# Veason-silverbullet/DIGAT

Hardware: AMD Instinct MI355X
Metric: MIND dev impressions scored/sec (AUC match not run) (higher is better)
Workload: dtype f32; 1 GPU; MIND-small default: --graph_encoder=DIGAT neighbors=3 hops=2 (N=10, U=67), d=400, graph_depth=3, fp32 dev inference; projection=auto -> fp16x3, N=10, U=67, d=400, graph_depth=3, news_num=65238, parallelism=dp1 (row shards, no data-path collective), ranks_in_process_group=1

## Files before the change

### digat_amd/csrc/digat_glue.inc

```

__global__ void __launch_bounds__(256) build_user_nodes_kernel(const float4* ue, const float4* topic, float4* Xu,
                                                               long B, int H, int C, int d4, const int* group, const uint8_t* rowmask = nullptr) {
    const long per_row = (long)(H + C) * d4;
    const long total = B * per_row;
    for (long i = (long)blockIdx.x * 256 + threadIdx.x; i < total; i += (long)gridDim.x * 256) {
        const long b = i / per_row;
        if (rowmask && rowmask[b] == 0) continue;
        const long rem = i - b * per_row;
        const long hist = (long)H * d4;
        const long src = group ? group[b] : b;
        Xu[i] = rem < hist ? ue[src * hist + rem] : topic[rem - hist];
    }
}

struct UserNodes3 { const float4* hist[3]; const float4* topic[3]; float4* dst[3]; };
__global__ void __launch_bounds__(256) build_user_nodes3_kernel(const UserNodes3 a, long B, int H, int C, int d4) {
    const int pl = blockIdx.y;
    const float4* ue = a.hist[pl];
    const float4* topic = a.topic[pl];
    float4* Xu = a.dst[pl];
    const long per_row = (long)(H + C) * d4;
    const long total = B * per_row;
    const long hist = (long)H * d4;
    for (long i = (long)blockIdx.x * 256 + threadIdx.x; i < total; i += (long)gridDim.x * 256) {
// ... 34 lines not shown
    unsigned long long col0 = 0ull, col1 = 0ull;
    unsigned long long own0[2] = {0ull, 0ull}, own1[2] = {0ull, 0ull};
    bool has0 = false, has1 = false;
    bool empty_row = false;
    int nz = 0;
    constexpr int RB = 8;
    for (int i0 = 0; i0 < U; i0 += RB) {
        uint8_t v0[RB], v1[RB];
#pragma unroll
        for (int r = 0; r < RB; ++r) {
            const uint8_t* row = A + (long)min(i0 + r, U - 1) * U;
            v0[r] = row[min(lane, U - 1)];
            v1[r] = row[min(lane + 64, U - 1)];
        }
#pragma unroll
        for (int r = 0; r < RB; ++r) {
            const int i = i0 + r;
            if (i >= U) break;
            unsigned long long m0 = __ballot(lane < U && v0[r] != 0), m1 = __ballot(lane + 64 < U && v1[r] != 0);
            nz += __popcll(m0) + __popcll(m1);
            empty_row |= (m0 | m1) == 0ull;
            if (twin && lane == (i & 63)) { own0[i >> 6] = m0; own1[i >> 6] = m1; }
            if (i < 64) m0 &= ~(1ull << i); else m1 &= ~(1ull << (i - 64));
            col0 |= m0; col1 |= m1;
            const bool has = (m0 | m1) != 0ull;
            if (lane == (i & 63)) { if (i < 64) has0 = has; else has1 = has; }
        }
    }
    const bool all_live = empty_row;
    int count = 0, last = 0;
    bool lv2[2] = {false, false};
#pragma unroll
    for (int h = 0; h < 2; ++h) {
        const int i = lane + 64 * h;
        bool live = false;
        if (i < U) {
            live = all_live || (h ? has1 : has0) || (((h ? col1 : col0) >> lane) & 1ull);
            if (i < H) {
                const long c = cat_idx[(long)b * H + i];
                live |= !any_cat || (c >= 0 && c < C1 && cat_mask[(long)b * C1 + c] != 0);
            }
            flags[(long)b * U + i] = live ? 1 : 0;
        }
        lv2[h] = live;
        count += __popcll(__ballot(live));
        const unsigned long long hm = __ballot(live && i < H);
        if (hm) last = 64 * h + 64 - __builtin_clzll(hm);
    }
    if (lane == 0) cnt[b] = count;
    if (lane == 0 && hlast) hlast[b] = last;
    if (twin) {
        int before[2] = {0, 0};
        unsigned word[2] = {0xFFFFFF00u | (unsigned)lane, 0xFFFFFF00u | (unsigned)(lane + 64)};
        unsigned long long rem0 = __ballot(lv2[0]), rem1 = __ballot(lv2[1]);
        while (rem0 | rem1) {
            const int hj = rem0 ? 0 : 1, lj = rem0 ? __builtin_ctzll(rem0) : __builtin_ctzll(rem1);
            const unsigned lo0 = (unsigned)__builtin_amdgcn_readlane((int)(unsigned)(hj ? own0[1] : own0[0]), lj);
            const unsigned hi0 = (unsigned)__builtin_amdgcn_readlane((int)(unsigned)((hj ? own0[1] : own0[0]) >> 32), lj);
            const unsigned lo1 = (unsigned)__builtin_amdgcn_readlane((int)(unsigned)(hj ? own1[1] : own1[0]), lj);
            const unsigned hi1 = (unsigned)__builtin_amdgcn_readlane((int)(unsigned)((hj ? own1[1] : own1[0]) >> 32), lj);
            const unsigned long long r0 = ((unsigned long long)hi0 << 32) | lo0, r1 = ((unsigned long long)hi1 << 32) | lo1;
            const bool e0 = lv2[0] && own0[0] == r0 && own1[0] == r1, e1 = lv2[1] && own0[1] == r0 && own1[1] == r1;
            const unsigned long long g0 = __ballot(e0), g1 = __ballot(e1);
            const unsigned long long below = (1ull << lane) - 1ull, above = lane == 63 ? 0ull : ~((2ull << lane) - 1ull);
            if (e0) {
                before[0] = __popcll(g0 & below);
                unsigned long long a0 = g0 & above, a1 = g1;
#pragma unroll
                for (int k = 1; k < TWIN_R; ++k) {
                    int j = -1;
                    if (a0) { j = __builtin_ctzll(a0); a0 &= a0 - 1ull; }
                    else if (a1) { j = 64 + __builtin_ctzll(a1); a1 &= a1 - 1ull; }
                    if (j >= 0) word[0] = (word[0] & ~(0xFFu << (8 * k))) | ((unsigned)j << (8 * k));
                }
            }
            if (e1) {
                before[1] = __popcll(g0) + __popcll(g1 & below);
                unsigned long long a1 = g1 & above;
#pragma unroll
                for (int k = 1; k < TWIN_R; ++k) {
                    if (a1) { const int j = 64 + __builtin_ctzll(a1); a1 &= a1 - 1ull; word[1] = (word[1] & ~(0xFFu << (8 * k))) | ((unsigned)j << (8 * k)); }
                }
            }
            rem0 &= ~g0; rem1 &= ~g1;
        }
        int leads = 0;
#pragma unroll
        for (int h = 0; h < 2; ++h) {
            const int i = lane + 64 * h;
            const bool lead = lv2[h] && (before[h] % TWIN_R) == 0;
            if (i < U) {
                twin[(long)b * U + i] = lead ? word[h] : 0xFFFFFFFFu;
                tflags[(long)b * U + i] = lead ? 1 : 0;
            }
            leads += __popcll(__ballot(lead));
        }
        if (lane == 0) tcnt[b] = leads;
    }
    if (entries && lane == 0) entries[b] = nz + (all_live ? U : 0);
    if (bflags) {
        int bc = 0;
        for (int c0 = 0; c0 < C1; c0 += 64) {
            const int c = c0 + lane;
            const bool bl = c < C1 && (!any_cat || cat_mask[(long)b * C1 + c] != 0);
            if (c < C1) bflags[(long)b * C1 + c] = bl ? 1 : 0;
            bc += __popcll(__ballot(bl));
        }
        if (lane == 0) bcnt[b] = bc;
    }
}

struct LiveExpand {
    const uint8_t* flags_g; const unsigned* twin_g; const uint8_t* tflags_g; const uint8_t* bflags_g;
    const int* cnt_g; const int* entries_g; const int* hlast_g; const int* bcnt_g; const int* tcnt_g;
    uint8_t* flags; unsigned* twin; uint8_t* tflags; uint8_t* bflags;
    int* cnt; int* entries; int* hlast; int* bcnt; int* tcnt;
};
__global__ void __launch_bounds__(256) live_expand_kernel(const LiveExpand a, const int* row_group, int B, int U, int C1) {
    const int lane = threadIdx.x & 63, wave = threadIdx.x >> 6;
    const int b = blockIdx.x * 4 + wave;
    if (b >= B) return;
    const long g = __builtin_amdgcn_readfirstlane(row_group[b]);
    if (a.flags_g == a.flags && g == b) return;
    for (int i = lane; i < U; i += 64) {
        a.flags[(long)b * U + i] = a.flags_g[g * U + i];
        if (a.twin) { a.twin[(long)b * U + i] = a.twin_g[g * U + i]; a.tflags[(long)b * U + i] = a.tflags_g[g * U + i]; }
    }
    if (a.bflags) for (int c = lane; c < C1; c += 64) a.bflags[(long)b * C1 + c] = a.bflags_g[g * C1 + c];
    if (lane == 0) {
        a.cnt[b] = a.cnt_g[g];
        if (a.hlast) a.hlast[b] = a.hlast_g[g];
        if (a.bcnt) a.bcnt[b] = a.bcnt_g[g];
        if (a.tcnt) a.tcnt[b] = a.tcnt_g[g];
        if (a.entries) a.entries[b] = a.entries_g[g];
    }
}

__global__ void __launch_bounds__(1024) sparse_decide_kernel(const int* entries, int B, int n, int per_node, int* flag) {
// ... 296 lines not shown
```

### digat_amd/csrc/digat_kernels.hip

```cpp
#include <hip/hip_runtime.h>
#include <stdint.h>
#include <string.h>
#include <stdlib.h>
#include <atomic>
#include <initializer_list>
#include <mutex>
#include <unordered_map>
#include <utility>

#include "../../include/digat_hip.h"
#include "digat_encoder_plan.h"

typedef float v4f __attribute__((ext_vector_type(4)));

#define DIGAT_CHECK_LAUNCH()                                   \
    do {                                                       \
        if (hipGetLastError() != hipSuccess) return DIGAT_ERR_LAUNCH; \
    } while (0)

static inline size_t align_up(size_t v, size_t a) { return (v + a - 1) / a * a; }
struct Arena {
    char* base; size_t cap, used; bool ok;
    Arena() : base(nullptr), cap(SIZE_MAX), used(0), ok(true) {}
    Arena(void* p, size_t n) : base((char*)p), cap(n), used(0), ok(p != nullptr) {}
// ... 65 lines not shown
    v += dpp_mov<0x141>(v);
    v += dpp_mov<0x140>(v);
#if DIGAT_WAVE_REDUCE_BCAST
    asm("s_nop 1\n\tv_add_f32_dpp %0, %0, %0 row_bcast:15 row_mask:0xa bank_mask:0xf\n\ts_nop 1\n\t"
        "v_add_f32_dpp %0, %0, %0 row_bcast:31 row_mask:0xc bank_mask:0xf\n\ts_nop 1" : "+v"(v));
    return lane_bcast(v, 63);
#else
    return (lane_bcast(v, 0) + lane_bcast(v, 16)) + (lane_bcast(v, 32) + lane_bcast(v, 48));
#endif
}
__device__ __forceinline__ float wave_max(float v) {
    v = fmaxf(v, dpp_mov<0xB1>(v));
    v = fmaxf(v, dpp_mov<0x4E>(v));
    v = fmaxf(v, dpp_mov<0x141>(v));
    v = fmaxf(v, dpp_mov<0x140>(v));
#if DIGAT_WAVE_REDUCE_BCAST
    asm("s_nop 1\n\tv_max_f32_dpp %0, %0, %0 row_bcast:15 row_mask:0xa bank_mask:0xf\n\ts_nop 1\n\t"
        "v_max_f32_dpp %0, %0, %0 row_bcast:31 row_mask:0xc bank_mask:0xf\n\ts_nop 1" : "+v"(v));
    return lane_bcast(v, 63);
#else
    return fmaxf(fmaxf(lane_bcast(v, 0), lane_bcast(v, 16)), fmaxf(lane_bcast(v, 32), lane_bcast(v, 48)));
#endif
}

__device__ __forceinline__ void lds_dma16(const float* gsrc, unsigned lds_byte_addr) {
    unsigned keep;
    asm volatile("s_mov_b32 %0, m0\n\ts_mov_b32 m0, %2\n\ts_nop 0\n\tglobal_load_lds_dwordx4 %1, off\n\ts_mov_b32 m0, %0"
                 : "=&s"(keep) : "v"(gsrc), "s"(lds_byte_addr) : "memory");
}
__device__ __forceinline__ void lds_dma16_s(const void* sbase_any, unsigned voff, unsigned lds_byte_addr) {
    const unsigned long long bits = (unsigned long long)(uintptr_t)sbase_any;
    const void* sbase = (const void*)(uintptr_t)(((unsigned long long)(unsigned)__builtin_amdgcn_readfirstlane((int)(bits >> 32)) << 32) |
                                                 (unsigned long long)(unsigned)__builtin_amdgcn_readfirstlane((int)bits));
    asm volatile("s_mov_b32 m0, %2\n\ts_nop 0\n\tglobal_load_lds_dwordx4 %0, %1" : : "v"(voff), "s"(sbase), "s"(lds_byte_addr) : "memory");
}
template <int N>
__device__ __forceinline__ void wait_vmcnt_imm() {
    __builtin_amdgcn_s_waitcnt((N & 15) | (7 << 4) | (15 << 8) | ((N >> 4) << 14));
}
__device__ __forceinline__ void wait_vmcnt(int n) {
    switch (n) {
        case 0: asm volatile("s_waitcnt vmcnt(0)" ::: "memory"); break;
        case 1: asm volatile("s_waitcnt vmcnt(1)" ::: "memory"); break;
        case 2: asm volatile("s_waitcnt vmcnt(2)" ::: "memory"); break;
        case 3: asm volatile("s_waitcnt vmcnt(3)" ::: "memory"); break;
        case 4: asm volatile("s_waitcnt vmcnt(4)" ::: "memory"); break;
        case 5: asm volatile("s_waitcnt vmcnt(5)" ::: "memory"); break;
        case 6: asm volatile("s_waitcnt vmcnt(6)" ::: "memory"); break;
        default: asm volatile("s_waitcnt vmcnt(4)" ::: "memory"); break;
    }
}

#ifndef DIGAT_TWIN_R
#define DIGAT_TWIN_R 2
#endif
__device__ __forceinline__ float leaky02_uniform(float e) {
    const float t = 0.2f * e;
    float r;
    asm("v_max_f32 %0, %1, %2" : "=v"(r) : "s"(e), "v"(t));
    return r;
}
__device__ __forceinline__ unsigned hash32(unsigned x) {
    x ^= x >> 16; x *= 0x7feb352dU; x ^= x >> 15; x *= 0x846ca68bU; x ^= x >> 16;
    return x;
}
__host__ __device__ __forceinline__ unsigned drop_threshold(float p) { return (unsigned)(p * 4294967296.0); }
__device__ __forceinline__ bool drop_keep(unsigned seed, long e, unsigned thr) {
    return hash32((unsigned)e * 0x9E3779B9U + hash32(seed + (unsigned)(e >> 32))) >= thr;
}
constexpr int TWIN_R = DIGAT_TWIN_R;
#include "digat_gemm.inc"
#include "digat_xattn.inc"
#include "digat_context.inc"
#include "digat_ctxfused.inc"
#include "digat_glue.inc"

extern "C" {

int digat_version(void) { return DIGAT_ABI_VERSION; }

const char* digat_error_string(int code) {
    switch (code) {
        case DIGAT_OK: return "ok";
        case DIGAT_ERR_ARG: return "bad argument (null pointer or negative size)";
        case DIGAT_ERR_SHAPE: return "unsupported shape (d % 4 != 0, graph larger than DIGAT_MAX_NODES, depth too large)";
        case DIGAT_ERR_WORKSPACE: return "workspace too small";
        case DIGAT_ERR_LAUNCH: return "HIP kernel launch failed";
        default: return "unknown error";
    }
}

int digat_linear_f32(const float* x, int64_t ldx, const float* w, const float* b, float* y, int64_t ldy,
                     int M, int N, int K, void* stream) {
    if (!x || !w || !y || M < 0 || N <= 0 || K <= 0) return DIGAT_ERR_ARG;
    if (K % 4 || ldx % 4) return DIGAT_ERR_SHAPE;
    return launch_gemm(gemm_plain(x, ldx, w, b, y, ldy, M, N, K, 0), (hipStream_t)stream);
}

struct XattnWs { float *h, *P, *Q, *r, *alpha; };
static XattnWs xattn_carve(Arena& a, int B, int n, int d) {
    const size_t nd = (size_t)B * n * d;
    XattnWs w{};
    w.h = a.take<float>(3 * nd);
    if (w.h) { w.P = w.h + nd; w.Q = w.P + nd; }
    w.r = a.take<float>((size_t)B * d);
    w.alpha = a.take<float>((size_t)B * n * n);
    return w;
}
size_t digat_xattn_workspace_bytes(int B, int n, int d) { Arena a; xattn_carve(a, B, n, d); return a.used; }

int digat_xattn_pairwise_fwd(const float* Pr, const float* Q, const float* h, const float* X,
                             const float* a, const uint8_t* A, float* out, float* alpha,
                             int B, int n, int d, void* stream) {
    if (!Pr || !Q || !h || !X || !a || !A || !out || !alpha) return DIGAT_ERR_ARG;
    return launch_xattn_pairwise(Pr, Q, h, X, a, A, out, alpha, B, n, d, (hipStream_t)stream);
}

struct TwinLists { const unsigned* word; const int* list; const int* count; };

struct XattnOpts {
    const void* wsplit = nullptr;
    const int* rowidx = nullptr; const int* nrows_dev = nullptr; const uint8_t* live = nullptr;
    int sparse_mode = DIGAT_XATTN_DENSE; const int* sparse_flag = nullptr;
// ... 512 lines not shown
```

### digat_amd/csrc/digat_xattn.inc

```

struct ScoreArgs {
    const float* P;
    const float* Q; const float* a; const uint8_t* A; float* alpha;
    float* s_out;
    const uint8_t* live;
    const int* qgroup;
    const float* radd;
    const int64_t* bindex;
    const float* agg_h; const float* agg_x; float* agg_out;
    int B, n, d, d4;
    int NT, SN, CC4, nchunks, RB;
    int img_slots;
    int ring_slots;
    int ninstr;
    int am_off;
    int a_off;
    int tl_off;
    int ld_off;
    int pm_off;
    const int* skip_if;
    uint8_t* amask; float* adrop; float drop_p; unsigned drop_seed;
};
constexpr int XA_RING = 3;
constexpr int XA_KMAX = 4;
// ... 966 lines not shown
#pragma unroll
        for (int u = 0; u < U; ++u) acc[r][u] = f4_zero();
    {
        unsigned long long m0 = m[0], m1 = m[1];
        while (m0 | m1) {
            int j[NBR], cnt = 0;
#pragma unroll
            for (int t = 0; t < NBR; ++t) {
                if (m0) { j[t] = __builtin_ctzll(m0); m0 &= m0 - 1ull; ++cnt; }
                else if (m1) { j[t] = 64 + __builtin_ctzll(m1); m1 &= m1 - 1ull; ++cnt; }
                else j[t] = j[0];
            }
            float4 hv[NBR][U];
#pragma unroll
            for (int t = 0; t < NBR; ++t)
#pragma unroll
                for (int u = 0; u < U; ++u) hv[t][u] = (Hb + (long)j[t] * d4)[c4l[u]];
#pragma unroll
            for (int t = 0; t < NBR; ++t) {
                if (t < cnt) {
#pragma unroll
                    for (int r = 0; r < R; ++r) {
                        if (r < nr) {
                            const float w = j[t] < 64 ? lane_bcast(al[r][0], j[t]) : lane_bcast(al[r][1], j[t] - 64);
#pragma unroll
                            for (int u = 0; u < U; ++u) {
                                acc[r][u].x = fmaf(w, hv[t][u].x, acc[r][u].x); acc[r][u].y = fmaf(w, hv[t][u].y, acc[r][u].y);
                                acc[r][u].z = fmaf(w, hv[t][u].z, acc[r][u].z); acc[r][u].w = fmaf(w, hv[t][u].w, acc[r][u].w);
                            }
                        }
                    }
                }
            }
        }
    }
#pragma unroll
    for (int r = 0; r < R; ++r) {
        if (r < nr) {
            float4* Oi = reinterpret_cast<float4*>(g.out) + (rho + (long)r * n) * d4;
#pragma unroll
            for (int u = 0; u < U; ++u) {
                const int c4 = lane + 64 * u;
                if (c4 < d4) {
                    const float4 x = xin[u];
                    const float4 o = make_float4(fmaxf(acc[r][u].x, 0.f) + x.x, fmaxf(acc[r][u].y, 0.f) + x.y,
                                                 fmaxf(acc[r][u].z, 0.f) + x.z, fmaxf(acc[r][u].w, 0.f) + x.w);
                    Oi[c4] = o;
                }
            }
        }
    }
}

template <int U, int R>
__device__ __forceinline__ void xattn_sparse_twin_chunk(const SparseArgs& g, const long rho, const unsigned word, const uint8_t ab0, const uint8_t ab1,
                                                        const int lane) {
    constexpr int NBR = DIGAT_SPARSE_NBR;
    const int n = g.n, d4 = g.d4;
    const long b = rho / n;
    int mem[R], nr = 0;
#pragma unroll
    for (int r = 0; r < R; ++r) {
        const int mi = (int)((word >> (8 * r)) & 0xFFu);
        const bool ok = mi != 0xFF && (g.centre_limit <= 0 || mi < g.centre_limit);
        mem[r] = ok ? mi : mem[0];
        nr += ok ? 1 : 0;
        if (r == 0 && !ok) return;
    }
    const float4* a4 = reinterpret_cast<const float4*>(g.a);
    float4 av[U], q[R][U];
    unsigned c4l[U];
#pragma unroll
    for (int u = 0; u < U; ++u) {
        const int c4 = min(lane + 64 * u, d4 - 1);
        c4l[u] = (unsigned)c4;
        const float4 aa = a4[c4];
        av[u] = lane + 64 * u < d4 ? aa : f4_zero();
#pragma unroll
        for (int r = 0; r < R; ++r) q[r][u] = reinterpret_cast<const float4*>(g.Q)[(b * n + mem[r]) * d4 + c4];
    }
    const float4* Pb = reinterpret_cast<const float4*>(g.P) + b * n * d4;
    const float4* Hb = reinterpret_cast<const float4*>(g.h) + b * n * d4;
    unsigned long long m[2];
    m[0] = __ballot(lane < n && ab0 != 0);
    m[1] = __ballot(lane + 64 < n && ab1 != 0);
    const int deg = __popcll(m[0]) + __popcll(m[1]);
    float al[R][2];
    if (deg == 0) {
        m[0] = n >= 64 ? ~0ull : ((1ull << n) - 1ull);
        m[1] = n > 64 ? (n >= 128 ? ~0ull : ((1ull << (n - 64)) - 1ull)) : 0ull;
        const float w = 1.f / (float)n;
#pragma unroll
        for (int r = 0; r < R; ++r) { al[r][0] = lane < n ? w : 0.f; al[r][1] = lane + 64 < n ? w : 0.f; }
    } else if (deg == 1) {
#pragma unroll
        for (int r = 0; r < R; ++r) { al[r][0] = ((m[0] >> lane) & 1ull) ? 1.f : 0.f; al[r][1] = ((m[1] >> lane) & 1ull) ? 1.f : 0.f; }
    } else {
        float sc[R][2];
#pragma unroll
        for (int r = 0; r < R; ++r) { sc[r][0] = -INFINITY; sc[r][1] = -INFINITY; }
        unsigned long long m0 = m[0], m1 = m[1];
        while (m0 | m1) {
            int j[NBR], cnt = 0;
#pragma unroll
            for (int t = 0; t < NBR; ++t) {
                if (m0) { j[t] = __builtin_ctzll(m0); m0 &= m0 - 1ull; ++cnt; }
                else if (m1) { j[t] = 64 + __builtin_ctzll(m1); m1 &= m1 - 1ull; ++cnt; }
                else j[t] = j[0];
            }
            float4 p[NBR][U];
#pragma unroll
            for (int t = 0; t < NBR; ++t)
#pragma unroll
                for (int u = 0; u < U; ++u) p[t][u] = (Pb + (long)j[t] * d4)[c4l[u]];
#pragma unroll
            for (int t = 0; t < NBR; ++t) {
                if (t < cnt) {
#pragma unroll
                    for (int r = 0; r < R; ++r) {
                        if (r < nr) {
                            float part = 0.f;
#pragma unroll
                            for (int u = 0; u < U; ++u) {
                                const float4 pk = p[t][u];
                                part = fmaf(av[u].x, fmaxf(pk.x + q[r][u].x, 0.f), part);
                                part = fmaf(av[u].y, fmaxf(pk.y + q[r][u].y, 0.f), part);
                                part = fmaf(av[u].z, fmaxf(pk.z + q[r][u].z, 0.f), part);
                                part = fmaf(av[u].w, fmaxf(pk.w + q[r][u].w, 0.f), part);
                            }
                            const float e = wave_sum(part);
                            const float lk = leaky02_uniform(e);
                            if (lane == (j[t] & 63)) { if (j[t] < 64) sc[r][0] = lk; else sc[r][1] = lk; }
                        }
                    }
                }
            }
        }
#pragma unroll
        for (int r = 0; r < R; ++r) {
            const float mx = wave_max(fmaxf(sc[r][0], sc[r][1]));
            const float e0 = sc[r][0] > -INFINITY ? expf(sc[r][0] - mx) : 0.f;
            const float e1 = sc[r][1] > -INFINITY ? expf(sc[r][1] - mx) : 0.f;
            const float inv = wave_sum(e0 + e1);
            al[r][0] = e0 / inv;
            al[r][1] = e1 / inv;
        }
    }
    float4 xin[R][U];
    {
        unsigned xo[U];
#pragma unroll
        for (int u = 0; u < U; ++u) { xo[u] = c4l[u]; asm volatile("" : "+v"(xo[u]) : "v"(al[0][0])); }
#pragma unroll
        for (int u = 0; u < U; ++u) xin[0][u] = reinterpret_cast<const float4*>(g.X)[(b * n + mem[0]) * d4 + xo[u]];
    }
    float4 acc[R][U];
#pragma unroll
    for (int r = 0; r < R; ++r)
#pragma unroll
        for (int u = 0; u < U; ++u) acc[r][u] = f4_zero();
    {
        unsigned long long m0 = m[0], m1 = m[1];
        while (m0 | m1) {
            int j[NBR], cnt = 0;
#pragma unroll
            for (int t = 0; t < NBR; ++t) {
                if (m0) { j[t] = __builtin_ctzll(m0); m0 &= m0 - 1ull; ++cnt; }
                else if (m1) { j[t] = 64 + __builtin_ctzll(m1); m1 &= m1 - 1ull; ++cnt; }
                else j[t] = j[0];
            }
            float4 hv[NBR][U];
#pragma unroll
            for (int t = 0; t < NBR; ++t)
#pragma unroll
                for (int u = 0; u < U; ++u) hv[t][u] = (Hb + (long)j[t] * d4)[c4l[u]];
#pragma unroll
            for (int t = 0; t < NBR; ++t) {
                if (t < cnt) {
#pragma unroll
                    for (int r = 0; r < R; ++r) {
                        if (r < nr) {
                            const float w = j[t] < 64 ? lane_bcast(al[r][0], j[t]) : lane_bcast(al[r][1], j[t] - 64);
#pragma unroll
                            for (int u = 0; u < U; ++u) {
                                acc[r][u].x = fmaf(w, hv[t][u].x, acc[r][u].x); acc[r][u].y = fmaf(w, hv[t][u].y, acc[r][u].y);
                                acc[r][u].z = fmaf(w, hv[t][u].z, acc[r][u].z); acc[r][u].w = fmaf(w, hv[t][u].w, acc[r][u].w);
                            }
                        }
                    }
                }
            }
        }
    }
    if (nr > 1) {
#pragma unroll
        for (int r = 1; r < R; ++r)
#pragma unroll
            for (int u = 0; u < U; ++u) xin[r][u] = reinterpret_cast<const float4*>(g.X)[(b * n + mem[r]) * d4 + c4l[u]];
    }
#pragma unroll
    for (int r = 0; r < R; ++r) {
        if (r < nr) {
            float4* Oi = reinterpret_cast<float4*>(g.out) + (b * n + mem[r]) * d4;
#pragma unroll
            for (int u = 0; u < U; ++u) {
                const int c4 = lane + 64 * u;
                if (c4 < d4) {
                    const float4 x = xin[r][u];
                    const float4 o = make_float4(fmaxf(acc[r][u].x, 0.f) + x.x, fmaxf(acc[r][u].y, 0.f) + x.y,
                                                 fmaxf(acc[r][u].z, 0.f) + x.z, fmaxf(acc[r][u].w, 0.f) + x.w);
                    Oi[c4] = o;
                }
            }
        }
    }
}

#ifndef DIGAT_TWIN_WAVES
#define DIGAT_TWIN_WAVES (DIGAT_TWIN_R <= 2 ? 5 : 4)
#endif
#ifndef DIGAT_TWIN_WPG
#define DIGAT_TWIN_WPG 4
#endif
template <int U, int R>
__global__ void __launch_bounds__(64 * DIGAT_TWIN_WPG, U <= 2 ? DIGAT_TWIN_WAVES : 1) xattn_sparse_twin_kernel(const SparseArgs g) {
    const int lane = threadIdx.x & 63, wave = __builtin_amdgcn_readfirstlane(threadIdx.x >> 6);
    if (g.exec_rows && g.exec_unit && blockIdx.x == 0 && threadIdx.x == 0) atomicAdd(g.exec_rows, (unsigned long long)*g.nrows_dev * g.exec_unit);
    unsigned blk = blockIdx.x;
    if (g.xcd_group > 0) {
        const unsigned Gx = (unsigned)g.xcd_group, w = blk / (8 * Gx), r = blk - w * 8 * Gx;
        blk = w * 8 * Gx + (r & 7) * Gx + (r >> 3);
    }
    const long count = *g.twcount;
    const long stride = (long)gridDim.x * DIGAT_TWIN_WPG;
    long k = (long)blk * DIGAT_TWIN_WPG + wave;
    if (k >= count) return;
    const int n = g.n;
    long rho = __builtin_amdgcn_readfirstlane(g.twlist[k]);
    unsigned word_v = g.twin[rho];
    uint8_t ab0 = g.A[rho * n + min(lane, n - 1)], ab1 = g.A[rho * n + min(lane + 64, n - 1)];
    int rho_next_v = g.twlist[min(k + stride, count - 1)];
    for (;;) {
        const long kn = k + stride;
        const bool more = kn < count;
        const long rho_n = more ? (long)__builtin_amdgcn_readfirstlane(rho_next_v) : rho;
        const unsigned word_n = g.twin[rho_n];
        const uint8_t ab0_n = g.A[rho_n * n + min(lane, n - 1)], ab1_n = g.A[rho_n * n + min(lane + 64, n - 1)];
        rho_next_v = g.twlist[min(kn + stride, count - 1)];
        xattn_sparse_twin_chunk<U, R>(g, rho, (unsigned)__builtin_amdgcn_readfirstlane((int)word_v), ab0, ab1, lane);
        if (!more) break;
        k = kn; rho = rho_n; word_v = word_n; ab0 = ab0_n; ab1 = ab1_n;
    }
}

__global__ void __launch_bounds__(1024) sparse_count_kernel(const int* rowidx, const int* nrows_dev, int n, int limit, unsigned unit, unsigned unit_nbr,
                                                            unsigned long long* out) {
    __shared__ int part[16], part2[16];
    const int total = *nrows_dev;
    int lo = 0, hi = 0;
    for (int k = blockIdx.x * 1024 + threadIdx.x; k < total; k += gridDim.x * 1024) { lo += (rowidx[k] % n) < limit; ++hi; }
    for (int o = 32; o > 0; o >>= 1) { lo += __shfl_xor(lo, o, 64); hi += __shfl_xor(hi, o, 64); }
    if ((threadIdx.x & 63) == 0) { part[threadIdx.x >> 6] = lo; part2[threadIdx.x >> 6] = hi; }
    __syncthreads();
    if (threadIdx.x == 0) {
        long t = 0, m = 0;
        for (int w = 0; w < 16; ++w) { t += part[w]; m += part2[w]; }
        if (m) atomicAdd(out, (unsigned long long)t * unit + (unsigned long long)(m - t) * unit_nbr);
    }
}

__global__ void __launch_bounds__(1024) sparse_l0_bytes_kernel(const uint8_t* live, const int* row_group, int B, int n, unsigned row_bytes,
                                                               unsigned long long* out) {
    __shared__ unsigned long long part[16];
    unsigned long long c = 0;
    for (int b = blockIdx.x * 1024 + threadIdx.x; b < B; b += gridDim.x * 1024) {
        int lv = 0;
        for (int i = 0; i < n; ++i) lv += live[(long)b * n + i] != 0;
        const bool first = b == 0 || row_group[b] != row_group[b - 1];
        c += (unsigned long long)lv * row_bytes + (first ? (unsigned long long)lv * (4ull * row_bytes + n) : 0ull);
    }
    for (int o = 32; o > 0; o >>= 1) c += __shfl_xor(c, o, 64);
    if ((threadIdx.x & 63) == 0) part[threadIdx.x >> 6] = c;
    __syncthreads();
    if (threadIdx.x == 0) {
        unsigned long long t = 0;
        for (int w = 0; w < 16; ++w) t += part[w];
        atomicAdd(out, t);
    }
}

static double sparse_bytes(const SparseArgs& g) {
    const double row = (double)g.d4 * 16;
    if (g.rowidx) return row + (g.radd ? (double)g.B * row : 0.0);
    double bytes = (double)g.B * g.n * g.n + row + (g.radd ? (double)g.B * row : 0.0);
    const double rows_b = (double)g.B * g.n, rows_g = (double)(g.group && g.G > 0 ? g.G : g.B) * g.n;
    bytes += 3.0 * rows_g * row;
    bytes += (g.group && g.xgroup ? rows_g : rows_b) * row;
    bytes += rows_b * row;
    return bytes;
}
static int sparse_part(const SparseArgs& g) { return g.prof_part ? g.prof_part - 1 : (g.rowidx ? (g.group ? XPART_L0 : XPART_TWIN) : XPART_OTHER); }
static int sparse_prof_bytes(SparseArgs& g, hipStream_t st) {
    g.exec_rows = nullptr; g.exec_unit = 0;
    if (!g.rowidx || !g_prof.enabled || !((g_prof.kind_mask >> DIGAT_KERNEL_XATTN) & 1u)) return DIGAT_OK;
    const unsigned row = (unsigned)g.d4 * 16;
    g.exec_rows = g_prof.rows_dev + 8 + sparse_part(g);
    const unsigned unit = g.pq16 == 2 ? (unsigned)(3.5 * row + 2.0 * 4 * (g.d4 / 20) + g.n) : (g.pq16 ? 4u : 5u) * row + (unsigned)g.n;
    if (g.group && g.live && !g.prof_part) {
        hipLaunchKernelGGL(sparse_l0_bytes_kernel, dim3((g.B + 1023) / 1024), dim3(1024), 0, st, g.live, g.group, g.B, g.n, row, g.exec_rows);
        DIGAT_CHECK_LAUNCH();
    } else if (g.centre_limit > 0) {
        hipLaunchKernelGGL(sparse_count_kernel, dim3(64), dim3(1024), 0, st, g.rowidx, g.nrows_dev, g.n, g.centre_limit, unit,
                           g.pq16 ? row + row / (g.pq16 == 2 ? 4 : 2) : 2 * row, g.exec_rows);
        DIGAT_CHECK_LAUNCH();
    } else {
        g.exec_unit = unit;
    }
    return DIGAT_OK;
}

#ifdef DIGAT_SPARSE_TIMERS
static unsigned long long* g_sparse_timers = nullptr;
extern "C" int digat_debug_sparse_timers(double* out9) {
    if (!g_sparse_timers || !out9) return DIGAT_ERR_ARG;
    unsigned long long h[9];
    if (hipDeviceSynchronize() != hipSuccess || hipMemcpy(h, g_sparse_timers, sizeof(h), hipMemcpyDeviceToHost) != hipSuccess) return DIGAT_ERR_LAUNCH;
    for (int k = 0; k < 9; ++k) out9[k] = (double)h[k];
    (void)hipMemset(g_sparse_timers, 0, 16 * 8);
    return DIGAT_OK;
}
#endif
static int launch_sparse(const SparseArgs& g_in, hipStream_t st) {
    SparseArgs g = g_in;
    if (g.n > 128 || g.d4 > 256) return DIGAT_ERR_SHAPE;
    { const int rcp = sparse_prof_bytes(g, st); if (rcp) return rcp; }
    ProfScope prof(DIGAT_KERNEL_XATTN, sparse_bytes(g), st, 0.0, sparse_part(g));
    unsigned blocks = (unsigned)(((long)g.B * g.n + 3) / 4);
    if (g.run_if && blocks > 2048u) blocks = 2048u;
    constexpr int SPARSE_XCD_GROUP = 16;
    g.xcd_group = SPARSE_XCD_GROUP;
#ifdef DIGAT_SPARSE_TIMERS
    if (!g_sparse_timers && hipMalloc((void**)&g_sparse_timers, 16 * 8) == hipSuccess) (void)hipMemset(g_sparse_timers, 0, 16 * 8);
    g.timers = g.rowidx ? g_sparse_timers : nullptr;
#endif
    blocks = (blocks + 8u * g.xcd_group - 1) / (8u * g.xcd_group) * (8u * g.xcd_group);
    if (g.twin && g.twlist && g.twcount && g.rowidx && !g.pq16 && !g.radd && !g.group && !g.run_if && !g.fill_flags && g.d4 <= 128) {
        constexpr unsigned TWIN_GRID_CAP = 8192;
        if (blocks > TWIN_GRID_CAP) blocks = TWIN_GRID_CAP;
        blocks = (blocks * 4 + DIGAT_TWIN_WPG - 1) / DIGAT_TWIN_WPG;
        if (g.d4 <= 64) hipLaunchKernelGGL((xattn_sparse_twin_kernel<1, TWIN_R>), dim3(blocks), dim3(64 * DIGAT_TWIN_WPG), 0, st, g);
        else hipLaunchKernelGGL((xattn_sparse_twin_kernel<2, TWIN_R>), dim3(blocks), dim3(64 * DIGAT_TWIN_WPG), 0, st, g);
        DIGAT_CHECK_LAUNCH();
        return DIGAT_OK;
    }
    if (g.pq16 == 2) {
        if (g.radd || g.d4 % 20 || g.ld8 < 4 * g.d4 + 4 * (g.d4 / 20) || (g.ld8 & 7)) return DIGAT_ERR_SHAPE;
        if (g.d4 <= 64) hipLaunchKernelGGL((xattn_sparse_kernel<1, 2, false>), dim3(blocks), dim3(256), 0, st, g);
        else if (g.d4 <= 128) hipLaunchKernelGGL((xattn_sparse_kernel<2, 2, false>), dim3(blocks), dim3(256), 0, st, g);
        else hipLaunchKernelGGL((xattn_sparse_kernel<4, 2, false>), dim3(blocks), dim3(256), 0, st, g);
    } else if (g.pq16) {
        if (g.radd || (g.d4 & 1)) return DIGAT_ERR_SHAPE;
        if (g.d4 <= 64) hipLaunchKernelGGL((xattn_sparse_kernel<1, 1, false>), dim3(blocks), dim3(256), 0, st, g);
        else if (g.d4 <= 128) hipLaunchKernelGGL((xattn_sparse_kernel<2, 1, false>), dim3(blocks), dim3(256), 0, st, g);
        else hipLaunchKernelGGL((xattn_sparse_kernel<4, 1, false>), dim3(blocks), dim3(256), 0, st, g);
    } else if (g.radd) {
        if (g.d4 <= 64) hipLaunchKernelGGL((xattn_sparse_kernel<1, 0, true>), dim3(blocks), dim3(256), 0, st, g);
        else if (g.d4 <= 128) hipLaunchKernelGGL((xattn_sparse_kernel<2, 0, true>), dim3(blocks), dim3(256), 0, st, g);
        else hipLaunchKernelGGL((xattn_sparse_kernel<4, 0, true>), dim3(blocks), dim3(256), 0, st, g);
    } else {
        if (g.d4 <= 64) hipLaunchKernelGGL((xattn_sparse_kernel<1, 0, false>), dim3(blocks), dim3(256), 0, st, g);
        else if (g.d4 <= 128) hipLaunchKernelGGL((xattn_sparse_kernel<2, 0, false>), dim3(blocks), dim3(256), 0, st, g);
        else hipLaunchKernelGGL((xattn_sparse_kernel<4, 0, false>), dim3(blocks), dim3(256), 0, st, g);
    }
    DIGAT_CHECK_LAUNCH();
    return DIGAT_OK;
}

#ifndef DIGAT_L0_ROWS
#define DIGAT_L0_ROWS 4
#endif
constexpr int SPARSE_L0_ROWS = DIGAT_L0_ROWS;
static bool sparse_l0_ok(const SparseArgs& g) {
    return g.group && g.xgroup && g.radd && g.rowidx && g.nrows_dev && g.live && !g.run_if && !g.pq16 && !g.fill_flags && !g.centre_limit &&
           g.n <= 128 && g.d4 <= 128;
}
static int launch_sparse_l0(const SparseArgs& g_in, const uint8_t* lead, const int* list, const int* count, int G, hipStream_t st) {
    SparseL0Args a{g_in, lead, list, count};
    SparseArgs& g = a.g;
    { const int rcp = sparse_prof_bytes(g, st); if (rcp) return rcp; }
    ProfScope prof(DIGAT_KERNEL_XATTN, sparse_bytes(g), st, 0.0, XPART_L0);
    constexpr int L0_XCD_GROUP = 16;
    g.xcd_group = L0_XCD_GROUP;
    unsigned blocks = (unsigned)((((long)g.B / SPARSE_L0_ROWS + G) * g.n + 3) / 4);
    blocks = (blocks + 8u * g.xcd_group - 1) / (8u * g.xcd_group) * (8u * g.xcd_group);
    if (g.d4 <= 64) hipLaunchKernelGGL((xattn_sparse_l0_kernel<1, SPARSE_L0_ROWS>), dim3(blocks), dim3(256), 0, st, a);
    else hipLaunchKernelGGL((xattn_sparse_l0_kernel<2, SPARSE_L0_ROWS>), dim3(blocks), dim3(256), 0, st, a);
    DIGAT_CHECK_LAUNCH();
    return DIGAT_OK;
}

struct AggArgs {
    const float* alpha; const float* Hh; const float* X; float* out; int B, n, d, groups, sa;
    const uint8_t* live;
    const int* hgroup;
// ... 219 lines not shown
```

Measured before the change: 39100 impressions/s.

## Group non-history twin rows with differing adjacency and raise twin group size

Rows at index H and above (topic/candidate nodes) are now grouped into twin chunks regardless of adjacency equality and flagged with a high bit. A uniform-adjacency-free variant of the sparse twin chunk then computes per-row masks and degrees and scores the union of neighbours. TWIN_R goes from 2 to 4 so more rows share the loaded P/H neighbour rows. Loads switch to scalar-base plus vector-offset addressing, and the neighbour batch sizes become template parameters. The aim is more reuse of each neighbour fetch per wave, at the cost of extra register pressure and wasted work on neighbours that only some rows in the group use.

```diff
diff --git a/digat_amd/csrc/digat_glue.inc b/digat_amd/csrc/digat_glue.inc
--- a/digat_amd/csrc/digat_glue.inc
+++ b/digat_amd/csrc/digat_glue.inc
@@ -110,7 +110,32 @@
     if (twin) {
         int before[2] = {0, 0};
         unsigned word[2] = {0xFFFFFF00u | (unsigned)lane, 0xFFFFFF00u | (unsigned)(lane + 64)};
-        unsigned long long rem0 = __ballot(lv2[0]), rem1 = __ballot(lv2[1]);
+        const unsigned long long below = (1ull << lane) - 1ull, above = lane == 63 ? 0ull : ~((2ull << lane) - 1ull);
+        auto place = [&](const bool e0, const bool e1, const unsigned long long g0, const unsigned long long g1) {
+            if (e0) {
+                before[0] = __popcll(g0 & below);
+                unsigned long long a0 = g0 & above, a1 = g1;
+#pragma unroll
+                for (int k = 1; k < TWIN_R; ++k) {
+                    int j = -1;
+                    if (a0) { j = __builtin_ctzll(a0); a0 &= a0 - 1ull; }
+                    else if (a1) { j = 64 + __builtin_ctzll(a1); a1 &= a1 - 1ull; }
+                    if (j >= 0) word[0] = (word[0] & ~(0xFFu << (8 * k))) | ((unsigned)j << (8 * k));
+                }
+            }
+            if (e1) {
+                before[1] = __popcll(g0) + __popcll(g1 & below);
+                unsigned long long a1 = g1 & above;
+#pragma unroll
+                for (int k = 1; k < TWIN_R; ++k) {
+                    if (a1) { const int j = 64 + __builtin_ctzll(a1); a1 &= a1 - 1ull; word[1] = (word[1] & ~(0xFFu << (8 * k))) | ((unsigned)j << (8 * k)); }
+                }
+            }
+        };
+        const bool top0 = lv2[0] && lane >= H, top1 = lv2[1] && lane + 64 >= H;
+        const unsigned long long t0 = __ballot(top0), t1 = __ballot(top1);
+        place(top0, top1, t0, t1);
+        unsigned long long rem0 = __ballot(lv2[0]) & ~t0, rem1 = __ballot(lv2[1]) & ~t1;
         while (rem0 | rem1) {
             const int hj = rem0 ? 0 : 1, lj = rem0 ? __builtin_ctzll(rem0) : __builtin_ctzll(rem1);
             const unsigned lo0 = (unsigned)__builtin_amdgcn_readlane((int)(unsigned)(hj ? own0[1] : own0[0]), lj);
@@ -118,30 +143,13 @@
             const unsigned lo1 = (unsigned)__builtin_amdgcn_readlane((int)(unsigned)(hj ? own1[1] : own1[0]), lj);
             const unsigned hi1 = (unsigned)__builtin_amdgcn_readlane((int)(unsigned)((hj ? own1[1] : own1[0]) >> 32), lj);
             const unsigned long long r0 = ((unsigned long long)hi0 << 32) | lo0, r1 = ((unsigned long long)hi1 << 32) | lo1;
-            const bool e0 = lv2[0] && own0[0] == r0 && own1[0] == r1, e1 = lv2[1] && own0[1] == r0 && own1[1] == r1;
+            const bool e0 = lv2[0] && !top0 && own0[0] == r0 && own1[0] == r1, e1 = lv2[1] && !top1 && own0[1] == r0 && own1[1] == r1;
             const unsigned long long g0 = __ballot(e0), g1 = __ballot(e1);
-            const unsigned long long below = (1ull << lane) - 1ull, above = lane == 63 ? 0ull : ~((2ull << lane) - 1ull);
-            if (e0) {
-                before[0] = __popcll(g0 & below);
-                unsigned long long a0 = g0 & above, a1 = g1;
-#pragma unroll
-                for (int k = 1; k < TWIN_R; ++k) {
-                    int j = -1;
-                    if (a0) { j = __builtin_ctzll(a0); a0 &= a0 - 1ull; }
-                    else if (a1) { j = 64 + __builtin_ctzll(a1); a1 &= a1 - 1ull; }
-                    if (j >= 0) word[0] = (word[0] & ~(0xFFu << (8 * k))) | ((unsigned)j << (8 * k));
-                }
-            }
-            if (e1) {
-                before[1] = __popcll(g0) + __popcll(g1 & below);
-                unsigned long long a1 = g1 & above;
-#pragma unroll
-                for (int k = 1; k < TWIN_R; ++k) {
-                    if (a1) { const int j = 64 + __builtin_ctzll(a1); a1 &= a1 - 1ull; word[1] = (word[1] & ~(0xFFu << (8 * k))) | ((unsigned)j << (8 * k)); }
-                }
-            }
+            place(e0, e1, g0, g1);
             rem0 &= ~g0; rem1 &= ~g1;
         }
+        if (top0 && (word[0] >> 8) != 0xFFFFFFu) word[0] |= 0x80u;
+        if (top1 && (word[1] >> 8) != 0xFFFFFFu) word[1] |= 0x80u;
         int leads = 0;
 #pragma unroll
         for (int h = 0; h < 2; ++h) {
diff --git a/digat_amd/csrc/digat_kernels.hip b/digat_amd/csrc/digat_kernels.hip
--- a/digat_amd/csrc/digat_kernels.hip
+++ b/digat_amd/csrc/digat_kernels.hip
@@ -141,7 +141,13 @@
 }
 
 #ifndef DIGAT_TWIN_R
-#define DIGAT_TWIN_R 2
+#define DIGAT_TWIN_R 4
+#endif
+#ifndef DIGAT_TWIN_NBR
+#define DIGAT_TWIN_NBR 2
+#endif
+#ifndef DIGAT_TWIN_NBR_AGG
+#define DIGAT_TWIN_NBR_AGG DIGAT_TWIN_NBR
 #endif
 __device__ __forceinline__ float leaky02_uniform(float e) {
     const float t = 0.2f * e;
@@ -158,6 +164,7 @@
     return hash32((unsigned)e * 0x9E3779B9U + hash32(seed + (unsigned)(e >> 32))) >= thr;
 }
 constexpr int TWIN_R = DIGAT_TWIN_R;
+constexpr int TWIN_NBR = DIGAT_TWIN_NBR, TWIN_NBR_AGG = DIGAT_TWIN_NBR_AGG;
 #include "digat_gemm.inc"
 #include "digat_xattn.inc"
 #include "digat_context.inc"
diff --git a/digat_amd/csrc/digat_xattn.inc b/digat_amd/csrc/digat_xattn.inc
--- a/digat_amd/csrc/digat_xattn.inc
+++ b/digat_amd/csrc/digat_xattn.inc
@@ -1042,17 +1042,35 @@
     }
 }
 
-template <int U, int R>
+typedef float f4raw __attribute__((ext_vector_type(4)));
+__device__ __forceinline__ float4 row_piece(const float4* row, const unsigned byte_off) {
+    unsigned long long base = reinterpret_cast<unsigned long long>(row);
+    asm("" : "+s"(base));
+    unsigned off = byte_off;
+    asm volatile("" : "+v"(off));
+    const auto* gb = reinterpret_cast<const __attribute__((address_space(1))) char*>(base);
+    const f4raw v = *reinterpret_cast<const __attribute__((address_space(1))) f4raw*>(gb + off);
+    return make_float4(v[0], v[1], v[2], v[3]);
+}
+__device__ __forceinline__ void row_piece_store(float4* row, const unsigned byte_off, const float4 v) {
+    unsigned long long base = reinterpret_cast<unsigned long long>(row);
+    asm("" : "+s"(base));
+    unsigned off = byte_off;
+    asm volatile("" : "+v"(off));
+    auto* gb = reinterpret_cast<__attribute__((address_space(1))) char*>(base);
+    const f4raw w = {v.x, v.y, v.z, v.w};
+    *reinterpret_cast<__attribute__((address_space(1))) f4raw*>(gb + off) = w;
+}
+template <int U, int R, int NBR, int NBRA, bool UNI>
 __device__ __forceinline__ void xattn_sparse_twin_chunk(const SparseArgs& g, const long rho, const unsigned word, const uint8_t ab0, const uint8_t ab1,
                                                         const int lane) {
-    constexpr int NBR = DIGAT_SPARSE_NBR;
     const int n = g.n, d4 = g.d4;
     const long b = rho / n;
     int mem[R], nr = 0;
 #pragma unroll
     for (int r = 0; r < R; ++r) {
-        const int mi = (int)((word >> (8 * r)) & 0xFFu);
-        const bool ok = mi != 0xFF && (g.centre_limit <= 0 || mi < g.centre_limit);
+        const int mi = (int)((word >> (8 * r)) & (r == 0 ? 0x7Fu : 0xFFu));
+        const bool ok = (r == 0 || mi != 0xFF) && (g.centre_limit <= 0 || mi < g.centre_limit);
         mem[r] = ok ? mi : mem[0];
         nr += ok ? 1 : 0;
         if (r == 0 && !ok) return;
@@ -1060,36 +1078,46 @@
     const float4* a4 = reinterpret_cast<const float4*>(g.a);
     float4 av[U], q[R][U];
     unsigned c4l[U];
+    uint8_t mb[UNI ? R : 1][2];
+    if constexpr (UNI) {
+#pragma unroll
+        for (int r = 1; r < R; ++r) {
+            const uint8_t* Ar = g.A + (b * n + mem[r]) * n;
+            mb[r][0] = Ar[min(lane, n - 1)]; mb[r][1] = Ar[min(lane + 64, n - 1)];
+        }
+    }
 #pragma unroll
     for (int u = 0; u < U; ++u) {
-        const int c4 = min(lane + 64 * u, d4 - 1);
-        c4l[u] = (unsigned)c4;
-        const float4 aa = a4[c4];
+        c4l[u] = 16u * (unsigned)min(lane + 64 * u, d4 - 1);
+        const float4 aa = row_piece(a4, c4l[u]);
         av[u] = lane + 64 * u < d4 ? aa : f4_zero();
 #pragma unroll
-        for (int r = 0; r < R; ++r) q[r][u] = reinterpret_cast<const float4*>(g.Q)[(b * n + mem[r]) * d4 + c4];
+        for (int r = 0; r < R; ++r) q[r][u] = row_piece(reinterpret_cast<const float4*>(g.Q) + (b * n + mem[r]) * d4, c4l[u]);
     }
     const float4* Pb = reinterpret_cast<const float4*>(g.P) + b * n * d4;
     const float4* Hb = reinterpret_cast<const float4*>(g.h) + b * n * d4;
-    unsigned long long m[2];
-    m[0] = __ballot(lane < n && ab0 != 0);
-    m[1] = __ballot(lane + 64 < n && ab1 != 0);
-    const int deg = __popcll(m[0]) + __popcll(m[1]);
+    constexpr int RM = UNI ? R : 1;
+    unsigned long long mk[RM][2];
+    int deg[RM];
+    unsigned long long su[2] = {0ull, 0ull};
+#pragma unroll
+    for (int r = 0; r < RM; ++r) {
+        const uint8_t b0 = r == 0 ? ab0 : mb[r][0], b1 = r == 0 ? ab1 : mb[r][1];
+        const bool in = r < nr;
+        mk[r][0] = in ? __ballot(lane < n && b0 != 0) : 0ull;
+        mk[r][1] = in ? __ballot(lane + 64 < n && b1 != 0) : 0ull;
+        deg[r] = in ? __popcll(mk[r][0]) + __popcll(mk[r][1]) : 2;
+        if (deg[r] >= 2) { su[0] |= mk[r][0]; su[1] |= mk[r][1]; }
+    }
+    auto takes = [&](const int r, const int j, const bool scoring) -> bool {
+        if constexpr (UNI) return (!scoring || deg[r] >= 2) && ((j < 64 ? mk[r][0] >> j : mk[r][1] >> (j - 64)) & 1ull) != 0ull;
+        else return r < nr;
+    };
     float al[R][2];
-    if (deg == 0) {
-        m[0] = n >= 64 ? ~0ull : ((1ull << n) - 1ull);
-        m[1] = n > 64 ? (n >= 128 ? ~0ull : ((1ull << (n - 64)) - 1ull)) : 0ull;
-        const float w = 1.f / (float)n;
-#pragma unroll
-        for (int r = 0; r < R; ++r) { al[r][0] = lane < n ? w : 0.f; al[r][1] = lane + 64 < n ? w : 0.f; }
-    } else if (deg == 1) {
-#pragma unroll
-        for (int r = 0; r < R; ++r) { al[r][0] = ((m[0] >> lane) & 1ull) ? 1.f : 0.f; al[r][1] = ((m[1] >> lane) & 1ull) ? 1.f : 0.f; }
-    } else {
-        float sc[R][2];
-#pragma unroll
-        for (int r = 0; r < R; ++r) { sc[r][0] = -INFINITY; sc[r][1] = -INFINITY; }
-        unsigned long long m0 = m[0], m1 = m[1];
+#pragma unroll
+    for (int r = 0; r < R; ++r) { al[r][0] = -INFINITY; al[r][1] = -INFINITY; }
+    {
+        unsigned long long m0 = su[0], m1 = su[1];
         while (m0 | m1) {
             int j[NBR], cnt = 0;
 #pragma unroll
@@ -1102,13 +1130,13 @@
 #pragma unroll
             for (int t = 0; t < NBR; ++t)
 #pragma unroll
-                for (int u = 0; u < U; ++u) p[t][u] = (Pb + (long)j[t] * d4)[c4l[u]];
+                for (int u = 0; u < U; ++u) p[t][u] = row_piece(Pb + (long)j[t] * d4, c4l[u]);
 #pragma unroll
             for (int t = 0; t < NBR; ++t) {
                 if (t < cnt) {
 #pragma unroll
                     for (int r = 0; r < R; ++r) {
-                        if (r < nr) {
+                        if (takes(r, j[t], true)) {
                             float part = 0.f;
 #pragma unroll
                             for (int u = 0; u < U; ++u) {
@@ -1120,20 +1148,30 @@
                             }
                             const float e = wave_sum(part);
                             const float lk = leaky02_uniform(e);
-                            if (lane == (j[t] & 63)) { if (j[t] < 64) sc[r][0] = lk; else sc[r][1] = lk; }
+                            if (lane == (j[t] & 63)) { if (j[t] < 64) al[r][0] = lk; else al[r][1] = lk; }
                         }
                     }
                 }
             }
         }
-#pragma unroll
-        for (int r = 0; r < R; ++r) {
-            const float mx = wave_max(fmaxf(sc[r][0], sc[r][1]));
-            const float e0 = sc[r][0] > -INFINITY ? expf(sc[r][0] - mx) : 0.f;
-            const float e1 = sc[r][1] > -INFINITY ? expf(sc[r][1] - mx) : 0.f;
-            const float inv = wave_sum(e0 + e1);
-            al[r][0] = e0 / inv;
-            al[r][1] = e1 / inv;
+    }
+#pragma unroll
+    for (int r = 0; r < R; ++r) {
+        if (r < nr) {
+            const int rm = UNI ? r : 0;
+            if (deg[rm] == 0) {
+                const float w = 1.f / (float)n;
+                al[r][0] = lane < n ? w : 0.f; al[r][1] = lane + 64 < n ? w : 0.f;
+            } else if (deg[rm] == 1) {
+                al[r][0] = ((mk[rm][0] >> lane) & 1ull) ? 1.f : 0.f; al[r][1] = ((mk[rm][1] >> lane) & 1ull) ? 1.f : 0.f;
+            } else {
+                const float mx = wave_max(fmaxf(al[r][0], al[r][1]));
+                const float e0 = al[r][0] > -INFINITY ? expf(al[r][0] - mx) : 0.f;
+                const float e1 = al[r][1] > -INFINITY ? expf(al[r][1] - mx) : 0.f;
+                const float inv = wave_sum(e0 + e1);
+                al[r][0] = e0 / inv;
+                al[r][1] = e1 / inv;
+            }
         }
     }
     float4 xin[R][U];
@@ -1142,34 +1180,43 @@
 #pragma unroll
         for (int u = 0; u < U; ++u) { xo[u] = c4l[u]; asm volatile("" : "+v"(xo[u]) : "v"(al[0][0])); }
 #pragma unroll
-        for (int u = 0; u < U; ++u) xin[0][u] = reinterpret_cast<const float4*>(g.X)[(b * n + mem[0]) * d4 + xo[u]];
+        for (int u = 0; u < U; ++u) xin[0][u] = row_piece(reinterpret_cast<const float4*>(g.X) + (b * n + mem[0]) * d4, xo[u]);
     }
     float4 acc[R][U];
 #pragma unroll
     for (int r = 0; r < R; ++r)
 #pragma unroll
         for (int u = 0; u < U; ++u) acc[r][u] = f4_zero();
+    unsigned long long au[2] = {0ull, 0ull};
+#pragma unroll
+    for (int r = 0; r < RM; ++r) {
+        if (deg[r] == 0) {
+            mk[r][0] = n >= 64 ? ~0ull : ((1ull << n) - 1ull);
+            mk[r][1] = n > 64 ? (n >= 128 ? ~0ull : ((1ull << (n - 64)) - 1ull)) : 0ull;
+        }
+        au[0] |= mk[r][0]; au[1] |= mk[r][1];
+    }
     {
-        unsigned long long m0 = m[0], m1 = m[1];
+        unsigned long long m0 = au[0], m1 = au[1];
         while (m0 | m1) {
-            int j[NBR], cnt = 0;
-#pragma unroll
-            for (int t = 0; t < NBR; ++t) {
+            int j[NBRA], cnt = 0;
+#pragma unroll
+            for (int t = 0; t < NBRA; ++t) {
                 if (m0) { j[t] = __builtin_ctzll(m0); m0 &= m0 - 1ull; ++cnt; }
                 else if (m1) { j[t] = 64 + __builtin_ctzll(m1); m1 &= m1 - 1ull; ++cnt; }
                 else j[t] = j[0];
             }
-            float4 hv[NBR][U];
-#pragma unroll
-            for (int t = 0; t < NBR; ++t)
-#pragma unroll
-                for (int u = 0; u < U; ++u) hv[t][u] = (Hb + (long)j[t] * d4)[c4l[u]];
-#pragma unroll
-            for (int t = 0; t < NBR; ++t) {
+            float4 hv[NBRA][U];
+#pragma unroll
+            for (int t = 0; t < NBRA; ++t)
+#pragma unroll
+                for (int u = 0; u < U; ++u) hv[t][u] = row_piece(Hb + (long)j[t] * d4, c4l[u]);
+#pragma unroll
+            for (int t = 0; t < NBRA; ++t) {
                 if (t < cnt) {
 #pragma unroll
                     for (int r = 0; r < R; ++r) {
-                        if (r < nr) {
+                        if (takes(r, j[t], false)) {
                             const float w = j[t] < 64 ? lane_bcast(al[r][0], j[t]) : lane_bcast(al[r][1], j[t] - 64);
 #pragma unroll
                             for (int u = 0; u < U; ++u) {
@@ -1186,7 +1233,7 @@
 #pragma unroll
         for (int r = 1; r < R; ++r)
 #pragma unroll
-            for (int u = 0; u < U; ++u) xin[r][u] = reinterpret_cast<const float4*>(g.X)[(b * n + mem[r]) * d4 + c4l[u]];
+            for (int u = 0; u < U; ++u) xin[r][u] = row_piece(reinterpret_cast<const float4*>(g.X) + (b * n + mem[r]) * d4, c4l[u]);
     }
 #pragma unroll
     for (int r = 0; r < R; ++r) {
@@ -1194,12 +1241,11 @@
             float4* Oi = reinterpret_cast<float4*>(g.out) + (b * n + mem[r]) * d4;
 #pragma unroll
             for (int u = 0; u < U; ++u) {
-                const int c4 = lane + 64 * u;
-                if (c4 < d4) {
+                if (lane + 64 * u < d4) {
                     const float4 x = xin[r][u];
                     const float4 o = make_float4(fmaxf(acc[r][u].x, 0.f) + x.x, fmaxf(acc[r][u].y, 0.f) + x.y,
                                                  fmaxf(acc[r][u].z, 0.f) + x.z, fmaxf(acc[r][u].w, 0.f) + x.w);
-                    Oi[c4] = o;
+                    row_piece_store(Oi, c4l[u], o);
                 }
             }
         }
@@ -1207,12 +1253,12 @@
 }
 
 #ifndef DIGAT_TWIN_WAVES
-#define DIGAT_TWIN_WAVES (DIGAT_TWIN_R <= 2 ? 5 : 4)
+#define DIGAT_TWIN_WAVES 5
 #endif
 #ifndef DIGAT_TWIN_WPG
 #define DIGAT_TWIN_WPG 4
 #endif
-template <int U, int R>
+template <int U, int R, int NBR, int NBRA>
 __global__ void __launch_bounds__(64 * DIGAT_TWIN_WPG, U <= 2 ? DIGAT_TWIN_WAVES : 1) xattn_sparse_twin_kernel(const SparseArgs g) {
     const int lane = threadIdx.x & 63, wave = __builtin_amdgcn_readfirstlane(threadIdx.x >> 6);
     if (g.exec_rows && g.exec_unit && blockIdx.x == 0 && threadIdx.x == 0) atomicAdd(g.exec_rows, (unsigned long long)*g.nrows_dev * g.exec_unit);
@@ -1237,7 +1283,9 @@
         const unsigned word_n = g.twin[rho_n];
         const uint8_t ab0_n = g.A[rho_n * n + min(lane, n - 1)], ab1_n = g.A[rho_n * n + min(lane + 64, n - 1)];
         rho_next_v = g.twlist[min(kn + stride, count - 1)];
-        xattn_sparse_twin_chunk<U, R>(g, rho, (unsigned)__builtin_amdgcn_readfirstlane((int)word_v), ab0, ab1, lane);
+        const unsigned word = (unsigned)__builtin_amdgcn_readfirstlane((int)word_v);
+        if (word & 0x80u) xattn_sparse_twin_chunk<U, R, NBR, NBRA, true>(g, rho, word, ab0, ab1, lane);
+        else xattn_sparse_twin_chunk<U, R, NBR, NBRA, false>(g, rho, word, ab0, ab1, lane);
         if (!more) break;
         k = kn; rho = rho_n; word_v = word_n; ab0 = ab0_n; ab1 = ab1_n;
     }
@@ -1338,8 +1386,8 @@
         constexpr unsigned TWIN_GRID_CAP = 8192;
         if (blocks > TWIN_GRID_CAP) blocks = TWIN_GRID_CAP;
         blocks = (blocks * 4 + DIGAT_TWIN_WPG - 1) / DIGAT_TWIN_WPG;
-        if (g.d4 <= 64) hipLaunchKernelGGL((xattn_sparse_twin_kernel<1, TWIN_R>), dim3(blocks), dim3(64 * DIGAT_TWIN_WPG), 0, st, g);
-        else hipLaunchKernelGGL((xattn_sparse_twin_kernel<2, TWIN_R>), dim3(blocks), dim3(64 * DIGAT_TWIN_WPG), 0, st, g);
+        if (g.d4 <= 64) hipLaunchKernelGGL((xattn_sparse_twin_kernel<1, TWIN_R, TWIN_NBR, TWIN_NBR_AGG>), dim3(blocks), dim3(64 * DIGAT_TWIN_WPG), 0, st, g);
+        else hipLaunchKernelGGL((xattn_sparse_twin_kernel<2, TWIN_R, TWIN_NBR, TWIN_NBR_AGG>), dim3(blocks), dim3(64 * DIGAT_TWIN_WPG), 0, st, g);
         DIGAT_CHECK_LAUNCH();
         return DIGAT_OK;
     }
```

New measurement: 38840 impressions/s. About the same (-0.6%).
